# speedinghzl/DSRG

Measured on AMD Instinct MI355X. Metric: images/sec DSRG train step (VGG16 321x321, 21-class), higher is better.
Workload: dtype bf16 backbone (fp32 master weights) + f32/f64 supervision path

## Files before the change

dsrg_amd/_lib.py:

```python
import ctypes
import os

import torch

_HERE = os.path.dirname(os.path.abspath(__file__))
LIB_PATH = os.path.join(_HERE, os.environ.get("DSRG_LIB") or "libdsrg_hip.so")

OK, ERR_INVALID, ERR_HIP, ERR_UNSUPPORTED, ERR_NOMEM = 0, -1, -2, -3, -4


class DsrgError(RuntimeError):
    def __init__(self, code, msg):
        RuntimeError.__init__(self, "libdsrg_hip error %d: %s" % (code, msg))
        self.code = code


class CrfParams(ctypes.Structure):
    _fields_ = [("w_bilateral", ctypes.c_float), ("theta_alpha_x", ctypes.c_float),
                ("theta_alpha_y", ctypes.c_float), ("theta_beta_r", ctypes.c_float),
                ("theta_beta_g", ctypes.c_float), ("theta_beta_b", ctypes.c_float),
                ("w_gaussian", ctypes.c_float), ("theta_gamma_x", ctypes.c_float),
                ("theta_gamma_y", ctypes.c_float), ("n_iters", ctypes.c_int32)]

    @classmethod
# ... 61 lines not shown
    "dsrg_conv_igemm_residual_bf16": (_i, [_vp] * 6 + [_i] * 8 + [_vp]),
    "dsrg_conv_igemm_split_f32": (_i, [_vp, _vp, _vp, _vp] + [_i] * 8 + [_vp]),
    "dsrg_add_relu_bf16": (_i, [_vp, _vp, _vp, _sz, _vp]),
    "dsrg_relu_mask_bf16": (_i, [_vp, _vp, _vp, _vp, _sz, _vp]),
    "dsrg_bias_grad_bf16": (_i, [_vp, _vp, _vp, _i, ctypes.c_long, _i, _vp]),
    "dsrg_heads_forward_bf16": (_i, [_vp, _i, _vp, _vp, _vp, _i, _i, _i, _i, _vp]),
    "dsrg_conv3x3_direct_bf16": (_i, [_vp, _vp, _vp, _vp, _i, _i, _i, _i, _i, _i, _vp]),
    "dsrg_conv3x3_direct_dgrad_workspace": (_sz, [_i]),
    "dsrg_conv3x3_direct_dgrad_bf16": (_i, [_vp] * 6 + [_sz] + [_i] * 5 + [_vp]),
    "dsrg_conv_igemm_supported": (_i, [_i, _i, _i]),
    "dsrg_conv_igemm_bf16": (_i, [_vp, _vp, _vp, _vp, _vp, _i, _i, _i, _i, _i, _i, _i, _i, ctypes.c_float, ctypes.c_ulonglong, _vp, _sz,
                                  _vp]),
    "dsrg_conv_igemm_workspace": (_sz, []),
    "dsrg_conv_igemm_dgrad_workspace": (_sz, [_i] * 5),
    "dsrg_conv_igemm_dgrad_bf16": (_i, [_vp] * 6 + [_i] * 7 + [_f, _vp, _sz, _vp]),
    "dsrg_conv_igemm_workspace_status": (_i, [_vp, _vp, _vp]),
    "dsrg_pack_conv_weight_f32": (_i, [_vp, _vp, _vp, _i, _i, _i, _vp]),
    "dsrg_sgd_pack_f32": (_i, [_i] + [_vp] * 9 + [_f, _vp]),
    "dsrg_conv_igemm_wgrad_workspace": (_sz, [_i, _i, _i, _i, _i, _i, _i]),
    "dsrg_conv_igemm_wgrad_bf16": (_i, [_vp, _vp, _vp, _vp, _i, _vp, _sz, _i, _i, _i, _i, _i, _i, _i, _vp]),
    "dsrg_conv_igemm_backward_bf16": (_i, [_vp, _vp, _vp, _vp, _vp, _vp, _i, _vp, _f, _vp, ctypes.c_size_t, _vp, ctypes.c_size_t, _i, _i, _i, _i, _i, _i, _vp]),
    "dsrg_conv3x3_wgrad_workspace": (_sz, [_i, _i, _i, _i, _i]),
    "dsrg_conv3x3_wgrad_bf16": (_i, [_vp, _vp, _vp, _vp, _sz, _i, _i, _i, _i, _i, _vp]),
    "dsrg_conv3x3_wgrad_f32": (_i, [_vp, _vp, _vp, _vp, _sz, _i, _i, _i, _i, _i, _vp]),
    "dsrg_pack_conv_weight_direct_f32": (_i, [_vp, _vp, _vp, _i, _i, _vp]),
    "dsrg_heads_backward_chunks": (_i, [_i]),
    "dsrg_heads_backward_bf16": (_i, [_vp, _i, _vp, _vp, _vp, _sz, _vp, _vp, _i, _i, _i, _i, _vp]),
    "dsrg_heads_backward_relu_workspace": (_sz, [_i] * 3),
    "dsrg_heads_backward_relu_bf16": (_i, [_vp, _i, _vp, _vp, _vp, _sz, _vp, _vp, _f, _vp, _vp, _sz] + [_i] * 4 + [_vp]),
    "dsrg_maxpool3x3_fwd_bf16": (_i, [_vp, _vp, _vp, _i, _i, _i, _i, _i, _i, _i, _vp]),
    "dsrg_maxpool3x3_relu_fwd_bf16": (_i, [_vp, _vp, _vp, _i, _i, _i, _i, _i, _i, _i, _vp]),
    "dsrg_maxpool3x3_bwd_bf16": (_i, [_vp, _vp, _vp, _i, _i, _i, _i, _i, _i, _i, _vp]),
    "dsrg_maxpool3x3_bwd_relu_bf16": (_i, [_vp, _vp, _vp, _vp, _vp, _vp, _i, _i, _i, _i, _i, _i, _i, _vp]),
    "dsrg_supervision_step": (_i, [_vp, _i, _vp, _vp, _i, _i, _vp, _vp, _d, _d, ctypes.POINTER(CrfParams),
                                   _vp, _vp, _vp, _vp, _vp, _vp]),
}

_LIB = None


def lib():
    global _LIB
    if _LIB is None:
        if not os.path.exists(LIB_PATH):
            raise ImportError(
                "%s is missing — build it with `make -C dsrg_amd/csrc` (hipcc --offload-arch=gfx950) or "
                "`python -c 'import __graft_entry__ as g; g.build()'`.  There is no CPU fallback." % LIB_PATH)
        L = ctypes.CDLL(LIB_PATH)
        for name, (res, args) in SIGNATURES.items():
            fn = getattr(L, name)
            fn.restype = res
            fn.argtypes = args
        _LIB = L
    return _LIB


def check(rc):
    if rc != OK:
        raise DsrgError(rc, lib().dsrg_last_error().decode("utf-8", "replace"))


def require_gpu():
    if lib().dsrg_device_count() < 1:
        raise DsrgError(ERR_HIP, "no HIP device visible — the DSRG supervision kernels need an MI355X "
                                 "(gfx950); there is no CPU fallback")
```

dsrg_amd/backbone.py:

```python
import torch
import torch.nn as nn
import torch.nn.functional as F

import os as _os

from . import ops

_WGRAD_MIN_COUT = 512
_GEMM_DGRAD_MAX_MAP = 2048
_GEMM_WGRAD_MAX_MAP = 2048
_IGEMM_MIN_TILES = 64
_IGEMM = _os.environ.get("DSRG_IGEMM", "1") == "1"


def _bf16_run(x):
    return x.dtype == torch.bfloat16 or (torch.is_autocast_enabled() and torch.get_autocast_dtype("cuda") == torch.bfloat16)


def _im2col_gemm(x, weight, bias, dilation, relu, want_cols=False):
    B, C, H, W = x.shape
    cout, k = weight.shape[0], weight.shape[2]
    xn = x.permute(0, 2, 3, 1)
    if not xn.is_contiguous():
        xn = xn.contiguous()
# ... 132 lines not shown

class _GradLink:
    __slots__ = ("scale", "gb", "ptr", "version")

    def __init__(self):
        self.scale, self.gb, self.ptr, self.version = 1.0, None, 0, -1

    def leave(self, gx, gb):
        self.gb, self.ptr, self.version = gb, gx.data_ptr(), gx._version

    def take(self, g):
        gb, self.gb = self.gb, None
        if gb is None:
            return None
        if g.data_ptr() == self.ptr and g._version == self.version:
            return gb
        if self.scale != 1.0:
            raise RuntimeError("chain_input: the output of a conv + ReLU + Dropout node declared to have one consumer has several")
        return None


_FUSE_CHAIN = _os.environ.get("DSRG_FUSE_CHAIN", "1") != "0"


def _landed(g, slot):
    return g.detach() if (slot is not None and g is slot) else g


class _IgemmConvFn(torch.autograd.Function):

    @staticmethod
    def forward(ctx, k, dils, relu, drop_p, pool, n, links_in, links_out, *t):
        xs, ws, bs = t[:n], t[n:2 * n], t[2 * n:3 * n]
        xs = [x if x.dtype == torch.bfloat16 else x.bfloat16() for x in xs]
        packs_d = [None] * n
        fb = [b.detach().float().contiguous() for b in bs]
        if drop_p > 0.0 and not relu:
            raise ValueError("_IgemmConvFn: Dropout needs the ReLU in front of it")
        fused_drop = drop_p > 0.0
        scale = 256.0 / (256 - min(255, int(drop_p * 256.0 + 0.5))) if fused_drop else 1.0
        seed = ops.dropout_seed() if fused_drop else 0
        if links_in is not None and not all(lk is not None for lk in links_in):
            links_in = None
        if k == 3:
            need_d = any(ctx.needs_input_grad[8:8 + n]) and ops.conv_igemm_supported(ws[0].shape[0], ws[0].shape[1], 3)
            packs = [ops.pack_conv_weight_pair(w, True, need_d) for w in ws]
            packs_d = [p[1] for p in packs]
            outs = ops.conv_igemm(xs, [p[0] for p in packs], fb, dils, 3, relu, drop_p, seed)
        elif fused_drop:
            packs = [ops.pack_conv_weight_pair(w, True, links_in is not None and _FUSE_CHAIN) for w in ws]
            packs_d = [p[1] for p in packs]
            outs = ops.conv_igemm(xs, [p[0] for p in packs], fb, dils, 1, relu, drop_p, seed)
        else:
            outs = [_im2col_gemm(x, w.to(torch.bfloat16), b.to(torch.bfloat16), 1, relu) for x, w, b in zip(xs, ws, bs)]
        code, pooled = None, None
        if pool is not None:
            pooled, code = ops.maxpool3x3_fwd(outs[0], pool[0], pool[1], relu_input=True)
        ctx.save_for_backward(code, *xs, *ws, *(outs if (relu and pool is None) else ()))
        ctx.out_shape = tuple(outs[0].shape)
        ctx.gw_out = [getattr(w, "_dsrg_grad_out", None) for w in ws]
        ctx.packs_d = packs_d
        ctx.dils, ctx.relu, ctx.scale, ctx.pool, ctx.n, ctx.k = dils, relu, scale, pool, n, k
        ctx.links_in = links_in
        ctx.links_out = links_out if (relu and pool is None) else None
        if ctx.links_out is not None:
            for lk in ctx.links_out:
                lk.scale, lk.gb = scale, None
        return tuple(outs) if pool is None else (pooled,)

    @staticmethod
    def backward(ctx, *gs):
        n = ctx.n
        code, saved = ctx.saved_tensors[0], ctx.saved_tensors[1:]
        xs, ws, ys = saved[:n], saved[n:2 * n], saved[2 * n:] or (None,) * n
        cout, cin = ws[0].shape[0], ws[0].shape[1]
        gms, gbs = [], []
        cl = torch.channels_last
        for i, g in enumerate(gs):
            gm, gb = g, ctx.links_out[i].take(g) if ctx.links_out is not None else None
            if gb is None:
                gm, gb = _relu_bias_backward(g, ctx.pool, code, ctx.out_shape, ctx.relu, ys[i], ctx.scale)
            gms.append(gm); gbs.append(gb)
        need_x = [ctx.needs_input_grad[8 + i] for i in range(n)]
        gxs = [None] * n
        absorb = _FUSE_CHAIN and ctx.links_in is not None and all(need_x) and ops.conv_igemm_supported(cout, cin, ctx.k) and \
            cin >= 256 and all(x.is_contiguous(memory_format=cl) for x in xs)
        if n == 1 and ctx.k == 3 and need_x[0] and ops.conv_igemm_supported(cout, cin, 3) and \
                ops.conv_igemm_wgrad_supported(cin, cout, 3) and xs[0].is_contiguous(memory_format=cl):
            pd = ctx.packs_d[0] if ctx.packs_d[0] is not None else ops.pack_conv_weight(ws[0], for_dgrad=True)
            gx, gw, gb_below = ops.conv_igemm_backward(gms[0], pd, xs[0], ctx.dils[0], xs[0] if absorb else None,
                                                       ctx.links_in[0].scale if absorb else 1.0, gw_out=ctx.gw_out[0])
            if absorb:
                ctx.links_in[0].leave(gx, gb_below)
            return (None,) * 8 + (gx, _landed(gw, ctx.gw_out[0])) + tuple(gbs)
        if absorb:
            packs_d = [p if p is not None else ops.pack_conv_weight(w, for_dgrad=True) for p, w in zip(ctx.packs_d, ws)]
            gxs, gb_below = ops.conv_igemm_dgrad(gms, packs_d, list(xs), ctx.dils, ctx.k, ctx.links_in[0].scale)
            for lk, gx_, gb_ in zip(ctx.links_in, gxs, gb_below):
                lk.leave(gx_, gb_)
        if ctx.k == 1:
            for i in range(n):
                if absorb:
                    break
                if need_x[i]:
# ... 125 lines not shown
            if igemm:
                (out,) = _IgemmConvFn.apply(3, [self.dilation[0]], self.fuse_relu, p, node_pool, 1, [lin] if lin is not None else None,
                                            [lout] if lout is not None else None, x, self.weight, self.bias)
            elif direct:
                out = _DirectConvFn.apply(x, self.weight, self.bias, self.fuse_relu, node_pool, lin, lout)
            else:
                out = _ConvFn.apply(x, self.weight, self.bias, self.dilation[0], self.fuse_relu, self.gemm, p, node_pool, lin, lout)
            if lout is not None:
                out._dsrg_grad_link = lout
            return out if pool is None or in_node else _pool3x3(out, pool[0], pool[1])
        out = super().forward(x)
        out = F.relu(out) if self.fuse_relu else out
        out = F.dropout(out, p, True) if p > 0.0 else out
        return out if pool is None else _pool3x3(out, pool[0], pool[1])


class FusedReLU(nn.Identity):
    """placeholder that keeps the Sequential indices (and state_dict keys) of the conv/ReLU pairs: the ReLU itself
    runs inside the GemmConv2d in front of it"""


class FusedPool(nn.Identity):
    """placeholder for the max-pool layer that runs inside the GemmConv2d two slots in front of it (`fuse_pool`)"""


class FusedDropout(nn.Identity):
    """placeholder for the Dropout layer that runs inside the GemmConv2d two slots in front of it (`fuse_dropout`)"""


def _hip_pool_takes(x):
    return x.is_cuda and x.dtype == torch.bfloat16 and x.shape[1] % 8 == 0 and x.is_contiguous(memory_format=torch.channels_last)


class _MaxPool3x3Fn(torch.autograd.Function):
    @staticmethod
    def forward(ctx, x, stride, ceil_mode):
        out, code = ops.maxpool3x3_fwd(x, stride, ceil_mode)
        ctx.save_for_backward(code)
        ctx.in_shape, ctx.stride = x.shape, stride
        return out

    @staticmethod
    def backward(ctx, g):
        (code,) = ctx.saved_tensors
        return ops.maxpool3x3_bwd(g, code, ctx.in_shape, ctx.stride), None, None


class _AvgPool3x3Fn(torch.autograd.Function):
    @staticmethod
    def forward(ctx, x):
        return ops.avgpool3x3_s1(x)

    @staticmethod
    def backward(ctx, g):
        return ops.avgpool3x3_s1(g)


class AvgPool3x3(nn.AvgPool2d):

    def __init__(self):
        super().__init__(3, 1, 1)

    def forward(self, x):
        if _hip_pool_takes(x):
            return _AvgPool3x3Fn.apply(x)
        if x.is_cuda and x.dim() == 4 and not x.is_contiguous():
            x = x.contiguous()
        return super().forward(x)


class MaxPool3x3(nn.MaxPool2d):

    def __init__(self, stride, ceil_mode=False):
        super().__init__(3, stride, 1, ceil_mode=ceil_mode)

    def forward(self, x):
        return _pool3x3(x, self.stride, self.ceil_mode)

# ... 16 lines not shown
        cl = torch.channels_last
        ctx.links = links if (links is not None and all(lk is not None for lk in links) and
                              all(x.is_contiguous(memory_format=cl) for x in xs)) else None
        xs = [x.contiguous(memory_format=cl) for x in xs]
        weight = weight.contiguous()
        ctx.save_for_backward(weight, *xs)
        return ops.heads_forward(xs, weight, bias.contiguous())

    @staticmethod
    def backward(ctx, g):
        weight, *xs = ctx.saved_tensors
        n, O, K = weight.shape
        if _FUSE_CHAIN and ctx.links is not None and all(ctx.needs_input_grad[3:]):
            gxs, gw, gb_below = ops.heads_backward(xs, weight, g, True, ctx.links[0].scale)
            for i, lk in enumerate(ctx.links):
                lk.leave(gxs[i], gb_below[i])
        else:
            gxs, gw = ops.heads_backward(xs, weight, g, need_gx=any(ctx.needs_input_grad[3:]))
        gb1 = g.sum((0, 2, 3))
        return (None, gw, gb1.unsqueeze(0).expand(n, O).contiguous()) + (tuple(gxs) if gxs is not None else (None,) * n)


class _StackKernels(torch.autograd.Function):

    @staticmethod
    def forward(ctx, *ws):
        ctx.layouts = [(tuple(w.shape), tuple(w.stride())) for w in ws]
        return torch.stack([w.reshape(w.shape[0], w.shape[1]) for w in ws])

    @staticmethod
    def backward(ctx, g):
        return tuple(g[i].as_strided(shape, stride) if g[i].is_contiguous() else g[i].reshape(shape)
                     for i, (shape, stride) in enumerate(ctx.layouts))


class VGG16ASPP(nn.Module):

    def __init__(self, num_classes=21, dropout=0.5, gemm_convs=True):
        super().__init__()
        L = []
        p2 = (2, True)
        L += _conv_relu(3, 64) + _conv_relu(64, 64, pool=p2, chain=True)
        L += _conv_relu(64, 128, 1, gemm_convs) + _conv_relu(128, 128, 1, gemm_convs, pool=p2, chain=True)
        L += _conv_relu(128, 256, 1, gemm_convs) + _conv_relu(256, 256, 1, gemm_convs, chain=True) + \
            _conv_relu(256, 256, 1, gemm_convs, pool=p2, chain=True)
        g = gemm_convs
        L += _conv_relu(256, 512, 1, g) + _conv_relu(512, 512, 1, g, chain=True) + _conv_relu(512, 512, 1, g, chain=True) + [MaxPool3x3(1)]
        L += _conv_relu(512, 512, 2, g) + _conv_relu(512, 512, 2, g, chain=True) + _conv_relu(512, 512, 2, g, chain=True) + [MaxPool3x3(1)]
        L += [AvgPool3x3()]
        self.features = nn.Sequential(*L)
        self.branches = nn.ModuleList()
        for d in (6, 12, 18, 24):
            g = gemm_convs
            fc8 = GemmConv2d(1024, num_classes, 1, gemm=g)
            nn.init.normal_(fc8.weight, std=0.01)
            nn.init.zeros_(fc8.bias)
            self.branches.append(nn.Sequential(
                GemmConv2d(512, 1024, 3, padding=d, dilation=d, fuse_relu=True, gemm=g, fuse_dropout=dropout), FusedReLU(),
                FusedDropout(),
                GemmConv2d(1024, 1024, 1, fuse_relu=True, gemm=g, fuse_dropout=dropout), FusedReLU(), FusedDropout(), fc8))

    def forward(self, x):
        f = self.features(x)
        hs = []
        fc6 = [br[0] for br in self.branches]
        if len(fc6) <= 4 and all(_igemm_route(m, f, len(fc6)) and m.stride == (1, 1) and m.padding == m.dilation for m in fc6):
            p = fc6[0].fuse_dropout if self.training else 0.0
            n = len(fc6)
            links = [_GradLink() for _ in range(n)] if torch.is_grad_enabled() else None
            hs = list(_IgemmConvFn.apply(3, [m.dilation[0] for m in fc6], True, p, None, n, None, links, *([f] * n),
                                         *[m.weight for m in fc6], *[m.bias for m in fc6]))
            fc7 = [br[3] for br in self.branches]
            if all(isinstance(m, GemmConv2d) and m.kernel_size == (1, 1) and m.fuse_relu and m.bias is not None and m.gemm
                   and m.in_channels % 256 == 0 and m.out_channels % 256 == 0 for m in fc7):
                p7 = fc7[0].fuse_dropout if self.training else 0.0
                links7 = [_GradLink() for _ in range(n)] if torch.is_grad_enabled() else None
                hs = list(_IgemmConvFn.apply(1, [1] * n, True, p7, None, n, links, links7, *hs, *[m.weight for m in fc7],
                                             *[m.bias for m in fc7]))
                for h, lk in zip(hs, links7 or []):
                    h._dsrg_grad_link = lk
            else:
                for i, br in enumerate(self.branches):
                    for m in list(br)[1:-1]:
                        hs[i] = m(hs[i])
        else:
            for br in self.branches:
                h = f
                for m in list(br)[:-1]:
                    h = m(h)
                hs.append(h)
        heads = [br[-1] for br in self.branches]
        if hs[0].is_cuda and hs[0].dtype == torch.bfloat16 and len(hs) <= 4 and heads[0].out_channels <= 32 \
                and heads[0].in_channels % 256 == 0:
            w = _StackKernels.apply(*[m.weight for m in heads])
            b = torch.stack([m.bias for m in heads])
            links = [getattr(h, "_dsrg_grad_link", None) for h in hs]
            return _HeadsFn.apply(links, w.float(), b.float(), *hs)
        out = None
        with torch.autocast(device_type=hs[0].device.type, enabled=False):
            for m, h in zip(heads, hs):
                s = m(h.float())
                out = s if out is None else out + s
        return out

# ... 49 lines not shown
```

dsrg_amd/ops.py:

```python
import ctypes
import threading

import torch

from . import _lib
from ._lib import CrfParams, check


def _stream():
    return ctypes.c_void_p(torch.cuda.current_stream().cuda_stream)


def _ptr(t):
    return ctypes.c_void_p(t.data_ptr()) if t is not None else None


def _f32c(t, name):
    if not (t.is_cuda and t.dtype == torch.float32 and t.is_contiguous()):
        raise ValueError("%s must be a contiguous float32 CUDA tensor" % name)
    return t


_defer = [False]
_defer_keep = []
# ... 973 lines not shown
        return [gx[k].permute(0, 3, 1, 2) for k in range(n)], gw, gb
    check(L.dsrg_heads_backward_bf16(ptrs, n, _ptr(weight), _ptr(g), _ptr(gx), M * K * 2, _ptr(gw), _ptr(part), B, H * W, K, O,
                                     _stream()))
    return ([gx[k].permute(0, 3, 1, 2) for k in range(n)] if need_gx else None), gw


def maxpool3x3_out_size(n, stride, ceil_mode):
    num = n + 2 - 3
    o = (-(-num // stride) if ceil_mode else num // stride) + 1
    if (o - 1) * stride >= n + 1:
        o -= 1
    return o


def maxpool3x3_fwd(x, stride, ceil_mode, relu_input=False):
    B, C, H, W = x.shape
    OH, OW = maxpool3x3_out_size(H, stride, ceil_mode), maxpool3x3_out_size(W, stride, ceil_mode)
    out = torch.empty((B, C, OH, OW), dtype=x.dtype, device=x.device, memory_format=torch.channels_last)
    code = torch.empty((B, OH, OW, C), dtype=torch.uint8, device=x.device)
    fn = _lib.lib().dsrg_maxpool3x3_relu_fwd_bf16 if relu_input else _lib.lib().dsrg_maxpool3x3_fwd_bf16
    check(fn(_ptr(x), _ptr(out), _ptr(code), B, H, W, OH, OW, C, stride, _stream()))
    return out, code


def maxpool3x3_bwd(gout, code, in_shape, stride):
    B, C, H, W = in_shape
    OH, OW = gout.shape[2], gout.shape[3]
    gout = gout.contiguous(memory_format=torch.channels_last)
    gin = torch.empty((B, C, H, W), dtype=gout.dtype, device=gout.device, memory_format=torch.channels_last)
    check(_lib.lib().dsrg_maxpool3x3_bwd_bf16(_ptr(gout), _ptr(code), _ptr(gin), B, H, W, OH, OW, C, stride, _stream()))
    return gin


def maxpool3x3_bwd_relu(gout, code, relu_out, stride=2, gb_out=None):
    have_y = torch.is_tensor(relu_out)
    B, C, H, W = relu_out.shape if have_y else relu_out
    OH, OW = gout.shape[2], gout.shape[3]
    cl = torch.channels_last
    if stride != 2 or not (gout.is_cuda and gout.dtype == torch.bfloat16 and C % 8 == 0 and 256 % (C // 8) == 0) or (
            have_y and not (relu_out.is_cuda and relu_out.dtype == torch.bfloat16 and relu_out.is_contiguous(memory_format=cl))):
        raise ValueError("maxpool3x3_bwd_relu: stride 2, bf16 channels_last, channels / 8 a divisor of 256")
    gout = gout.contiguous(memory_format=cl)
    gin = torch.empty((B, C, H, W), dtype=torch.bfloat16, device=gout.device, memory_format=cl)
    gb = _dest(gb_out, (C,), torch.float32, gout.device)
    part = _partial_rows(gout.device, C)
    check(_lib.lib().dsrg_maxpool3x3_bwd_relu_bf16(_ptr(gout), _ptr(code), _ptr(relu_out) if have_y else None, _ptr(gin), _ptr(gb), _ptr(part),
                                                   _PARTIAL_BLOCKS, B, H, W, OH, OW, C, _stream()))
    return gin, gb


class DSRGSupervision(torch.autograd.Function):

    @staticmethod
    def forward(ctx, logits, images, labels, cues, th1, th2, scale_factor, maxiter, prepared=False):
        losses, grad, _ = supervision_step(logits.contiguous(), images, labels, cues, th1, th2, scale_factor, maxiter,
                                           prepared=prepared)
        ctx.save_for_backward(grad)
        ctx.mark_non_differentiable(losses)
        return losses.sum(), losses

    @staticmethod
    def backward(ctx, g_total, _g_losses):
        (grad,) = ctx.saved_tensors
        return grad * g_total, None, None, None, None, None, None, None, None


# ... 4 lines not shown
```

include/dsrg_hip.h:

```cpp
#ifndef DSRG_HIP_H
#define DSRG_HIP_H

#include <stddef.h>
#include <stdint.h>

#ifdef __cplusplus
extern "C" {
#endif

#pragma GCC visibility push(default)

#define DSRG_OK 0
#define DSRG_ERR_INVALID (-1)
#define DSRG_ERR_HIP (-2)
#define DSRG_ERR_UNSUPPORTED (-3)
#define DSRG_ERR_NOMEM (-4)

const char *dsrg_last_error(void);
int dsrg_device_count(void);
int dsrg_host_register(void *host, size_t bytes);
int dsrg_host_unregister(void *host);

typedef struct dsrg_crf_s *dsrg_crf_t;

// ... 134 lines not shown
                      float momentum, void *stream);
size_t dsrg_conv_igemm_wgrad_workspace(int ngroups, int B, int H, int W, int cin, int cout, int ksize);
int dsrg_conv_igemm_wgrad_bf16(const void *const *x_dev, const void *const *g_dev, void *const *gw_dev, const int *dilation,
                               int ngroups, void *workspace_dev, size_t workspace_bytes, int B, int H, int W, int cin, int cout,
                               int ksize, int out_bf16, void *stream);
int dsrg_conv_igemm_backward_bf16(const void *g_dev, const void *w_dgrad_dev, const void *x_dev, const void *mask_dev, void *gx_dev,
                                  float *gw_dev, int dilation, float *bias_grad_dev, float mask_scale, void *colsum_workspace_dev,
                                  size_t colsum_workspace_bytes, void *wgrad_workspace_dev, size_t wgrad_workspace_bytes, int B, int H,
                                  int W, int cin, int cout, int ksize, void *stream);
int dsrg_conv_igemm_backward_residual_bf16(const void *g_dev, const void *w_dgrad_dev, const void *x_dev, const void *mask_dev,
                                           const void *res_dev, void *gx_dev, float *gw_dev, const float *gw_scale_dev, int dilation,
                                           void *wgrad_workspace_dev, size_t wgrad_workspace_bytes, int B, int H, int W, int cin, int cout,
                                           int ksize, void *stream);
int dsrg_heads_forward_bf16(const void *const *x_dev, int n_branches, const float *w_dev, const float *bias_dev,
                            float *out_dev, int B, int HW, int K, int O, void *stream);
int dsrg_heads_backward_chunks(int M);
int dsrg_heads_backward_bf16(const void *const *x_dev, int n_branches, const float *w_dev, const float *g_dev,
                             void *gx_dev, size_t gx_branch_stride_bytes, float *gw_dev, float *partial_dev, int B,
                             int HW, int K, int O, void *stream);
size_t dsrg_heads_backward_relu_workspace(int n_branches, int M, int K);
int dsrg_heads_backward_relu_bf16(const void *const *x_dev, int n_branches, const float *w_dev, const float *g_dev,
                                  void *gx_dev, size_t gx_branch_stride_bytes, float *gw_dev, float *partial_dev,
                                  float relu_scale, float *bias_grad_dev, void *workspace_dev, size_t workspace_bytes, int B,
                                  int HW, int K, int O, void *stream);
int dsrg_maxpool3x3_fwd_bf16(const void *in_dev, void *out_dev, void *code_dev, int B, int H, int W, int OH, int OW, int C,
                             int stride, void *stream);
int dsrg_maxpool3x3_relu_fwd_bf16(const void *in_dev, void *out_dev, void *code_dev, int B, int H, int W, int OH, int OW, int C,
                                  int stride, void *stream);
int dsrg_maxpool3x3_bwd_bf16(const void *gout_dev, const void *code_dev, void *gin_dev, int B, int H, int W, int OH, int OW,
                             int C, int stride, void *stream);
int dsrg_maxpool3x3_bwd_relu_bf16(const void *gout_dev, const void *code_dev, const void *relu_out_dev, void *gin_dev,
                                  float *bias_grad_dev, float *partials_dev, int partial_blocks, int B, int H, int W, int OH,
                                  int OW, int C, void *stream);

int dsrg_supervision_step(dsrg_ctx_t ctx, int B, const float *logits_dev, const float *images_dev,
                          int img_h, int img_w, const float *labels_dev, const float *cues_dev,
                          double th1, double th2, const dsrg_crf_params *params,
                          float *losses_dev, float *grad_logits_dev,
                          float *probs_dev, float *seeds_dev, float *logq_dev, void *stream);

#pragma GCC visibility pop

#ifdef __cplusplus
}
#endif
#endif
```

Measured before the change: 1958.

## Fuse final stride-1 maxpool and avgpool with LDS-tiled kernels and branch-gradient sum

Adds LDS-tiled HIP kernels for the stride-1 3x3 maxpool, plus a fused maxpool-then-avgpool forward and backward for the end of the feature stack. In backward, the four ASPP branch input gradients are passed straight to the fused pool backward through a link object instead of being summed by autograd, so the separate sum and pool passes over HBM go away. The cost is extra bookkeeping that can fall back when a gradient was modified in place, plus LDS-size limits that trigger the old path.

```diff
diff --git a/dsrg_amd/_lib.py b/dsrg_amd/_lib.py
--- a/dsrg_amd/_lib.py
+++ b/dsrg_amd/_lib.py
@@ -117,6 +117,11 @@
     "dsrg_maxpool3x3_relu_fwd_bf16": (_i, [_vp, _vp, _vp, _i, _i, _i, _i, _i, _i, _i, _vp]),
     "dsrg_maxpool3x3_bwd_bf16": (_i, [_vp, _vp, _vp, _i, _i, _i, _i, _i, _i, _i, _vp]),
     "dsrg_maxpool3x3_bwd_relu_bf16": (_i, [_vp, _vp, _vp, _vp, _vp, _vp, _i, _i, _i, _i, _i, _i, _i, _vp]),
+    "dsrg_pool_chain_rows": (_i, []),
+    "dsrg_maxpool3x3_s1_tiled_fwd_bf16": (_i, [_vp, _vp, _vp, _i, _i, _i, _i, _vp]),
+    "dsrg_maxavg3x3_s1_fwd_bf16": (_i, [_vp, _vp, _vp, _i, _i, _i, _i, _vp]),
+    "dsrg_maxpool3x3_s1_tiled_bwd_bf16": (_i, [_vp, _vp, _vp, _i, _i, _i, _i, _vp]),
+    "dsrg_maxavg3x3_s1_bwd_bf16": (_i, [_vp, _vp, _vp, _vp, _i, _vp, _vp, _i, _i, _i, _i, _vp]),
     "dsrg_supervision_step": (_i, [_vp, _i, _vp, _vp, _i, _i, _vp, _vp, _d, _d, ctypes.POINTER(CrfParams),
                                    _vp, _vp, _vp, _vp, _vp, _vp]),
 }
diff --git a/dsrg_amd/backbone.py b/dsrg_amd/backbone.py
--- a/dsrg_amd/backbone.py
+++ b/dsrg_amd/backbone.py
@@ -188,6 +188,8 @@
     @staticmethod
     def forward(ctx, k, dils, relu, drop_p, pool, n, links_in, links_out, *t):
         xs, ws, bs = t[:n], t[n:2 * n], t[2 * n:3 * n]
+        ctx.extra = len(t) - 3 * n
+        ctx.sum_link = t[3 * n] if ctx.extra else None
         xs = [x if x.dtype == torch.bfloat16 else x.bfloat16() for x in xs]
         packs_d = [None] * n
         fb = [b.detach().float().contiguous() for b in bs]
@@ -226,6 +228,16 @@
 
     @staticmethod
     def backward(ctx, *gs):
+        res = _IgemmConvFn._backward(ctx, *gs)
+        n, lk = ctx.n, ctx.sum_link
+        gxs = res[8:8 + n]
+        if lk is not None and _POOL_CHAIN and n > 1 and all(g is not None and _hip_pool_takes(g) for g in gxs):
+            lk.leave(gxs)
+            res = res[:9] + (None,) * (n - 1) + res[8 + n:]
+        return res + (None,) * ctx.extra
+
+    @staticmethod
+    def _backward(ctx, *gs):
         n = ctx.n
         code, saved = ctx.saved_tensors[0], ctx.saved_tensors[1:]
         xs, ws, ys = saved[:n], saved[n:2 * n], saved[2 * n:] or (None,) * n
@@ -417,10 +429,16 @@
     return x.is_cuda and x.dtype == torch.bfloat16 and x.shape[1] % 8 == 0 and x.is_contiguous(memory_format=torch.channels_last)
 
 
+_POOL_CHAIN = _os.environ.get("DSRG_POOL_CHAIN", "1") != "0"
+
+
 class _MaxPool3x3Fn(torch.autograd.Function):
     @staticmethod
     def forward(ctx, x, stride, ceil_mode):
-        out, code = ops.maxpool3x3_fwd(x, stride, ceil_mode)
+        if stride == 1 and _POOL_CHAIN:
+            out, code = ops.maxpool3x3_s1_tiled_fwd(x, ctx.needs_input_grad[0])
+        else:
+            out, code = ops.maxpool3x3_fwd(x, stride, ceil_mode)
         ctx.save_for_backward(code)
         ctx.in_shape, ctx.stride = x.shape, stride
         return out
@@ -428,7 +446,48 @@
     @staticmethod
     def backward(ctx, g):
         (code,) = ctx.saved_tensors
+        if ctx.stride == 1 and _POOL_CHAIN and _hip_pool_takes(g):
+            return ops.maxpool3x3_s1_tiled_bwd(g, code), None, None
         return ops.maxpool3x3_bwd(g, code, ctx.in_shape, ctx.stride), None, None
+
+
+class _SumLink:
+    __slots__ = ("gs", "ptr", "version")
+
+    def __init__(self):
+        self.gs, self.ptr, self.version = None, 0, -1
+
+    def leave(self, gs):
+        self.gs, self.ptr, self.version = list(gs), gs[0].data_ptr(), gs[0]._version
+
+    def take(self, g):
+        gs, self.gs = self.gs, None
+        if gs is None:
+            return [g], True
+        if g.data_ptr() == self.ptr and g._version == self.version and g.shape == gs[0].shape and g.dtype == gs[0].dtype:
+            return gs, True
+        return [g] + gs[1:], False
+
+
+class _PoolChainFn(torch.autograd.Function):
+
+    @staticmethod
+    def forward(ctx, x, link):
+        out, code = ops.maxavg3x3_s1_fwd(x, ctx.needs_input_grad[0])
+        ctx.save_for_backward(code)
+        ctx.in_shape, ctx.link = x.shape, link
+        return out
+
+    @staticmethod
+    def backward(ctx, g):
+        (code,) = ctx.saved_tensors
+        gs, intact = ctx.link.take(g) if ctx.link is not None else ([g], True)
+        if intact and _POOL_CHAIN and all(_hip_pool_takes(t) for t in gs):
+            return ops.maxavg3x3_s1_bwd(gs, code), None
+        s = gs[0]
+        for t in gs[1:]:
+            s = s + t
+        return ops.maxpool3x3_bwd(ops.avgpool3x3_s1(s), code, ctx.in_shape, 1), None
 
 
 class _AvgPool3x3Fn(torch.autograd.Function):
@@ -511,6 +570,24 @@
     def backward(ctx, g):
         return tuple(g[i].as_strided(shape, stride) if g[i].is_contiguous() else g[i].reshape(shape)
                      for i, (shape, stride) in enumerate(ctx.layouts))
+
+
+class _Features(nn.Sequential):
+
+    def forward(self, x):
+        mods = list(self)
+        if not (_POOL_CHAIN and len(mods) >= 2 and isinstance(mods[-2], MaxPool3x3) and mods[-2].stride == 1
+                and isinstance(mods[-1], AvgPool3x3)):
+            return super().forward(x)
+        for m in mods[:-2]:
+            x = m(x)
+        if not _hip_pool_takes(x):
+            return mods[-1](mods[-2](x))
+        link = _SumLink() if (torch.is_grad_enabled() and x.requires_grad) else None
+        out = _PoolChainFn.apply(x, link)
+        if link is not None:
+            out._dsrg_sum_link = link
+        return out
 
 
 class VGG16ASPP(nn.Module):
@@ -527,7 +604,7 @@
         L += _conv_relu(256, 512, 1, g) + _conv_relu(512, 512, 1, g, chain=True) + _conv_relu(512, 512, 1, g, chain=True) + [MaxPool3x3(1)]
         L += _conv_relu(512, 512, 2, g) + _conv_relu(512, 512, 2, g, chain=True) + _conv_relu(512, 512, 2, g, chain=True) + [MaxPool3x3(1)]
         L += [AvgPool3x3()]
-        self.features = nn.Sequential(*L)
+        self.features = _Features(*L)
         self.branches = nn.ModuleList()
         for d in (6, 12, 18, 24):
             g = gemm_convs
@@ -547,8 +624,10 @@
             p = fc6[0].fuse_dropout if self.training else 0.0
             n = len(fc6)
             links = [_GradLink() for _ in range(n)] if torch.is_grad_enabled() else None
+            sum_link = getattr(f, "_dsrg_sum_link", None) if (_POOL_CHAIN and n > 1) else None
             hs = list(_IgemmConvFn.apply(3, [m.dilation[0] for m in fc6], True, p, None, n, None, links, *([f] * n),
-                                         *[m.weight for m in fc6], *[m.bias for m in fc6]))
+                                         *[m.weight for m in fc6], *[m.bias for m in fc6],
+                                         *([sum_link] if sum_link is not None else [])))
             fc7 = [br[3] for br in self.branches]
             if all(isinstance(m, GemmConv2d) and m.kernel_size == (1, 1) and m.fuse_relu and m.bias is not None and m.gemm
                    and m.in_channels % 256 == 0 and m.out_channels % 256 == 0 for m in fc7):
diff --git a/dsrg_amd/csrc/pool_chain.hip b/dsrg_amd/csrc/pool_chain.hip
--- /dev/null
+++ b/dsrg_amd/csrc/pool_chain.hip
@@ -0,0 +1,391 @@
+#include "common.h"
+#include <algorithm>
+
+#ifndef DSRG_POOL_ROWS
+#define DSRG_POOL_ROWS 8
+#endif
+
+namespace dsrg {
+namespace {
+
+constexpr int kPoolRows = DSRG_POOL_ROWS;
+constexpr int kSegRows = 4;
+constexpr int kMaxThreads = 1024;
+constexpr size_t kLdsLimit = 160 * 1024;
+
+__device__ __forceinline__ float lo16(uint32_t w) { return __uint_as_float(w << 16); }
+__device__ __forceinline__ float hi16(uint32_t w) { return __uint_as_float(w & 0xffff0000u); }
+__device__ __forceinline__ uint32_t to_bf16(float f) {
+    uint32_t u = __float_as_uint(f);
+    if ((u & 0x7fffffffu) > 0x7f800000u) return (u >> 16) | 0x40u;
+    return (u + 0x7fffu + ((u >> 16) & 1u)) >> 16;
+}
+__device__ __forceinline__ uint32_t pack2(float lo, float hi) { return to_bf16(lo) | (to_bf16(hi) << 16); }
+__device__ __forceinline__ uint32_t to_bf16_torch(float f) {
+    uint32_t u = __float_as_uint(f);
+    if (f != f) return 0x7fc0u;
+    return (u + 0x7fffu + ((u >> 16) & 1u)) >> 16;
+}
+__device__ __forceinline__ uint32_t add_pair(uint32_t a, uint32_t b) {
+    return to_bf16_torch(lo16(a) + lo16(b)) | (to_bf16_torch(hi16(a) + hi16(b)) << 16);
+}
+__device__ __forceinline__ uint4 add_vec(uint4 a, uint4 b) {
+    return make_uint4(add_pair(a.x, b.x), add_pair(a.y, b.y), add_pair(a.z, b.z), add_pair(a.w, b.w));
+}
+
+struct Tile {
+    int b, y0, y1;
+    int cg0, cga;
+    int H, W, C8;
+};
+__device__ __forceinline__ Tile make_tile(int H, int W, int C8, int CG) {
+    Tile t;
+    t.b = blockIdx.z;
+    t.y0 = blockIdx.x * kPoolRows;
+    t.y1 = min(H, t.y0 + kPoolRows);
+    t.cg0 = blockIdx.y * CG;
+    t.cga = min(CG, C8 - t.cg0);
+    t.H = H; t.W = W; t.C8 = C8;
+    return t;
+}
+
+template <typename T>
+__device__ __forceinline__ void stage_rows(T *lds, const T *__restrict__ g, const Tile &t, int ra, int rb, int base) {
+    ra = max(ra, 0); rb = min(rb, t.H);
+    const int lanes = blockDim.x / t.cga, c = threadIdx.x % t.cga, p0 = threadIdx.x / t.cga;
+    if (p0 >= lanes) return;
+    const int npix = (rb - ra) * t.W;
+    const T *src = g + ((size_t)t.b * t.H + ra) * t.W * t.C8 + t.cg0 + c;
+    T *dst = lds + (size_t)(ra - base) * t.W * t.cga + c;
+    int p = p0;
+    for (; p + 3 * lanes < npix; p += 4 * lanes) {
+        const T v0 = src[(size_t)p * t.C8], v1 = src[(size_t)(p + lanes) * t.C8];
+        const T v2 = src[(size_t)(p + 2 * lanes) * t.C8], v3 = src[(size_t)(p + 3 * lanes) * t.C8];
+        dst[p * t.cga] = v0; dst[(p + lanes) * t.cga] = v1; dst[(p + 2 * lanes) * t.cga] = v2; dst[(p + 3 * lanes) * t.cga] = v3;
+    }
+    for (; p < npix; p += lanes) dst[p * t.cga] = src[(size_t)p * t.C8];
+}
+
+__device__ __forceinline__ void stage_sum_rows(uint4 *lds, const uint4 *__restrict__ g0, const uint4 *__restrict__ g1,
+                                               const uint4 *__restrict__ g2, const uint4 *__restrict__ g3, int n, const Tile &t,
+                                               int ra, int rb, int base) {
+    ra = max(ra, 0); rb = min(rb, t.H);
+    const int lanes = blockDim.x / t.cga, c = threadIdx.x % t.cga, p0 = threadIdx.x / t.cga;
+    if (p0 >= lanes) return;
+    const int npix = (rb - ra) * t.W;
+    const size_t off = ((size_t)t.b * t.H + ra) * t.W * t.C8 + t.cg0 + c;
+    uint4 *dst = lds + (size_t)(ra - base) * t.W * t.cga + c;
+    for (int p = p0; p < npix; p += lanes) {
+        const size_t i = off + (size_t)p * t.C8;
+        uint4 s = g0[i];
+        if (n > 1) {
+            const uint4 a = g1[i];
+            if (n > 2) {
+                const uint4 b2 = g2[i];
+                if (n > 3) {
+                    const uint4 b3 = g3[i];
+                    s = add_vec(add_vec(add_vec(s, a), b2), b3);
+                } else {
+                    s = add_vec(add_vec(s, a), b2);
+                }
+            } else {
+                s = add_vec(s, a);
+            }
+        }
+        dst[p * t.cga] = s;
+    }
+}
+
+struct Task { int c, x, ys, ye; };
+__device__ __forceinline__ int task_count(const Tile &t, int ra, int rb) { return ((rb - ra + kSegRows - 1) / kSegRows) * t.W * t.cga; }
+__device__ __forceinline__ Task make_task(const Tile &t, int i, int ra, int rb) {
+    Task k;
+    k.c = i % t.cga;
+    const int q = i / t.cga;
+    k.x = q % t.W;
+    k.ys = ra + (q / t.W) * kSegRows;
+    k.ye = min(rb, k.ys + kSegRows);
+    return k;
+}
+
+struct RowMax { float v[8]; uint32_t c[8]; };
+__device__ __forceinline__ void row_max(const uint4 *row, int x, int W, int cga, int c, RowMax &r) {
+#pragma unroll
+    for (int k = 0; k < 8; ++k) { r.v[k] = -__builtin_inff(); r.c[k] = 0xffu; }
+#pragma unroll
+    for (int dx = 0; dx < 3; ++dx) {
+        const int xx = x - 1 + dx;
+        if (xx < 0 || xx >= W) continue;
+        const uint4 v = row[xx * cga + c];
+        const uint32_t w[4] = {v.x, v.y, v.z, v.w};
+#pragma unroll
+        for (int k = 0; k < 4; ++k) {
+            const float lo = lo16(w[k]), hi = hi16(w[k]);
+            if (lo > r.v[2 * k] || lo != lo || r.c[2 * k] == 0xffu) { r.v[2 * k] = lo; r.c[2 * k] = dx; }
+            if (hi > r.v[2 * k + 1] || hi != hi || r.c[2 * k + 1] == 0xffu) { r.v[2 * k + 1] = hi; r.c[2 * k + 1] = dx; }
+        }
+    }
+}
+__device__ __forceinline__ void fold_row(const RowMax &r, int dy, float *best, uint32_t *bc) {
+#pragma unroll
+    for (int k = 0; k < 8; ++k)
+        if (r.v[k] > best[k] || r.v[k] != r.v[k] || bc[k] == 0xffu) { best[k] = r.v[k]; bc[k] = 3 * dy + r.c[k]; }
+}
+
+template <bool TO_LDS>
+__device__ __forceinline__ void maxpool_rows(const uint4 *in_l, int in_base, const Tile &t, int ra, int rb, uint4 *out_g, uint4 *out_l,
+                                             int out_base, uint2 *code, int ca, int cb) {
+    const int W = t.W, cga = t.cga, H = t.H, ntask = task_count(t, ra, rb);
+    for (int i = threadIdx.x; i < ntask; i += blockDim.x) {
+        const Task k = make_task(t, i, ra, rb);
+        RowMax r0, r1, r2;
+        if (k.ys > 0) row_max(in_l + (size_t)(k.ys - 1 - in_base) * W * cga, k.x, W, cga, k.c, r0);
+        row_max(in_l + (size_t)(k.ys - in_base) * W * cga, k.x, W, cga, k.c, r1);
+        for (int y = k.ys; y < k.ye; ++y) {
+            if (y + 1 < H) row_max(in_l + (size_t)(y + 1 - in_base) * W * cga, k.x, W, cga, k.c, r2);
+            float best[8];
+            uint32_t bc[8];
+#pragma unroll
+            for (int j = 0; j < 8; ++j) { best[j] = -__builtin_inff(); bc[j] = 0xffu; }
+            if (y > 0) fold_row(r0, 0, best, bc);
+            fold_row(r1, 1, best, bc);
+            if (y + 1 < H) fold_row(r2, 2, best, bc);
+            const uint4 o = make_uint4(pack2(best[0], best[1]), pack2(best[2], best[3]), pack2(best[4], best[5]), pack2(best[6], best[7]));
+            const size_t gi = (((size_t)t.b * H + y) * W + k.x) * t.C8 + t.cg0 + k.c;
+            if (TO_LDS) out_l[((size_t)(y - out_base) * W + k.x) * cga + k.c] = o;
+            else out_g[gi] = o;
+            if (code && y >= ca && y < cb)
+                code[gi] = make_uint2(bc[0] | (bc[1] << 8) | (bc[2] << 16) | (bc[3] << 24), bc[4] | (bc[5] << 8) | (bc[6] << 16) | (bc[7] << 24));
+            r0 = r1; r1 = r2;
+        }
+    }
+}
+
+__device__ __forceinline__ void load_taps(const uint4 *row, int x, int W, int cga, int c, uint4 *w) {
+    if (x > 0) w[0] = row[(x - 1) * cga + c];
+    w[1] = row[x * cga + c];
+    if (x + 1 < W) w[2] = row[(x + 1) * cga + c];
+}
+__device__ __forceinline__ void load_taps(const uint2 *row, int x, int W, int cga, int c, uint2 *w) {
+    if (x > 0) w[0] = row[(x - 1) * cga + c];
+    w[1] = row[x * cga + c];
+    if (x + 1 < W) w[2] = row[(x + 1) * cga + c];
+}
+__device__ __forceinline__ void add_taps(const uint4 *w, bool left, bool right, float *acc) {
+#pragma unroll
+    for (int dx = 0; dx < 3; ++dx) {
+        if ((dx == 0 && !left) || (dx == 2 && !right)) continue;
+        const uint32_t u[4] = {w[dx].x, w[dx].y, w[dx].z, w[dx].w};
+#pragma unroll
+        for (int k = 0; k < 4; ++k) { acc[2 * k] += lo16(u[k]); acc[2 * k + 1] += hi16(u[k]); }
+    }
+}
+
+template <bool TO_LDS>
+__device__ __forceinline__ void avgpool_rows(const uint4 *in_l, int in_base, const Tile &t, int ra, int rb, uint4 *out_g, uint4 *out_l,
+                                             int out_base) {
+    const int W = t.W, cga = t.cga, H = t.H, ntask = task_count(t, ra, rb);
+    for (int i = threadIdx.x; i < ntask; i += blockDim.x) {
+        const Task k = make_task(t, i, ra, rb);
+        const bool left = k.x > 0, right = k.x + 1 < W;
+        uint4 w0[3], w1[3], w2[3];
+        w0[0] = w0[1] = w0[2] = w1[0] = w1[1] = w1[2] = w2[0] = w2[1] = w2[2] = make_uint4(0u, 0u, 0u, 0u);
+        if (k.ys > 0) load_taps(in_l + (size_t)(k.ys - 1 - in_base) * W * cga, k.x, W, cga, k.c, w0);
+        load_taps(in_l + (size_t)(k.ys - in_base) * W * cga, k.x, W, cga, k.c, w1);
+        for (int y = k.ys; y < k.ye; ++y) {
+            if (y + 1 < H) load_taps(in_l + (size_t)(y + 1 - in_base) * W * cga, k.x, W, cga, k.c, w2);
+            float acc[8] = {0.f, 0.f, 0.f, 0.f, 0.f, 0.f, 0.f, 0.f};
+            if (y > 0) add_taps(w0, left, right, acc);
+            add_taps(w1, left, right, acc);
+            if (y + 1 < H) add_taps(w2, left, right, acc);
+#pragma unroll
+            for (int j = 0; j < 8; ++j) acc[j] = acc[j] / 9.0f;
+            const uint4 o = make_uint4(pack2(acc[0], acc[1]), pack2(acc[2], acc[3]), pack2(acc[4], acc[5]), pack2(acc[6], acc[7]));
+            if (TO_LDS) out_l[((size_t)(y - out_base) * W + k.x) * cga + k.c] = o;
+            else out_g[(((size_t)t.b * H + y) * W + k.x) * t.C8 + t.cg0 + k.c] = o;
+#pragma unroll
+            for (int j = 0; j < 3; ++j) { w0[j] = w1[j]; w1[j] = w2[j]; }
+        }
+    }
+}
+
+__device__ __forceinline__ void gather_taps(const uint4 *g, const uint2 *cd, int dy, bool left, bool right, float *acc) {
+#pragma unroll
+    for (int dx = 0; dx < 3; ++dx) {
+        if ((dx == 0 && !right) || (dx == 2 && !left)) continue;
+        const uint4 gv = g[2 - dx];
+        const uint2 cv = cd[2 - dx];
+        const uint32_t want = 3 * dy + dx;
+        const uint32_t gw[4] = {gv.x, gv.y, gv.z, gv.w};
+#pragma unroll
+        for (int k = 0; k < 4; ++k) {
+            const uint32_t cw = k < 2 ? cv.x : cv.y;
+            const uint32_t c0 = (cw >> (16 * (k & 1))) & 0xffu, c1 = (cw >> (16 * (k & 1) + 8)) & 0xffu;
+            if (c0 == want) acc[2 * k] += lo16(gw[k]);
+            if (c1 == want) acc[2 * k + 1] += hi16(gw[k]);
+        }
+    }
+}
+
+__device__ __forceinline__ void maxpool_bwd_rows(const uint4 *g_l, const uint2 *c_l, int base, const Tile &t, int ra, int rb, uint4 *gin) {
+    const int W = t.W, cga = t.cga, H = t.H, ntask = task_count(t, ra, rb);
+    for (int i = threadIdx.x; i < ntask; i += blockDim.x) {
+        const Task k = make_task(t, i, ra, rb);
+        const bool left = k.x > 0, right = k.x + 1 < W;
+        uint4 g0[3], g1[3], g2[3];
+        uint2 c0[3], c1[3], c2[3];
+        g0[0] = g0[1] = g0[2] = g1[0] = g1[1] = g1[2] = g2[0] = g2[1] = g2[2] = make_uint4(0u, 0u, 0u, 0u);
+        c0[0] = c0[1] = c0[2] = c1[0] = c1[1] = c1[2] = c2[0] = c2[1] = c2[2] = make_uint2(0u, 0u);
+        if (k.ys > 0) {
+            load_taps(g_l + (size_t)(k.ys - 1 - base) * W * cga, k.x, W, cga, k.c, g0);
+            load_taps(c_l + (size_t)(k.ys - 1 - base) * W * cga, k.x, W, cga, k.c, c0);
+        }
+        load_taps(g_l + (size_t)(k.ys - base) * W * cga, k.x, W, cga, k.c, g1);
+        load_taps(c_l + (size_t)(k.ys - base) * W * cga, k.x, W, cga, k.c, c1);
+        for (int y = k.ys; y < k.ye; ++y) {
+            if (y + 1 < H) {
+                load_taps(g_l + (size_t)(y + 1 - base) * W * cga, k.x, W, cga, k.c, g2);
+                load_taps(c_l + (size_t)(y + 1 - base) * W * cga, k.x, W, cga, k.c, c2);
+            }
+            float acc[8] = {0.f, 0.f, 0.f, 0.f, 0.f, 0.f, 0.f, 0.f};
+            if (y + 1 < H) gather_taps(g2, c2, 0, left, right, acc);
+            gather_taps(g1, c1, 1, left, right, acc);
+            if (y > 0) gather_taps(g0, c0, 2, left, right, acc);
+            gin[(((size_t)t.b * H + y) * W + k.x) * t.C8 + t.cg0 + k.c] =
+                make_uint4(pack2(acc[0], acc[1]), pack2(acc[2], acc[3]), pack2(acc[4], acc[5]), pack2(acc[6], acc[7]));
+#pragma unroll
+            for (int j = 0; j < 3; ++j) { g0[j] = g1[j]; g1[j] = g2[j]; c0[j] = c1[j]; c1[j] = c2[j]; }
+        }
+    }
+}
+
+extern __shared__ uint4 pool_lds[];
+
+__global__ __launch_bounds__(kMaxThreads) void maxpool3x3_s1_tiled_fwd_kernel(const uint4 *__restrict__ in, uint4 *__restrict__ out,
+                                                                                uint2 *__restrict__ code, int H, int W, int C8, int CG) {
+    const Tile t = make_tile(H, W, C8, CG);
+    const int base = t.y0 - 1;
+    stage_rows(pool_lds, in, t, t.y0 - 1, t.y1 + 1, base);
+    __syncthreads();
+    maxpool_rows<false>(pool_lds, base, t, t.y0, t.y1, out, nullptr, 0, code, t.y0, t.y1);
+}
+
+__global__ __launch_bounds__(kMaxThreads) void maxavg3x3_s1_fwd_kernel(const uint4 *__restrict__ in, uint4 *__restrict__ out,
+                                                                         uint2 *__restrict__ code, int H, int W, int C8, int CG) {
+    const Tile t = make_tile(H, W, C8, CG);
+    const int base = t.y0 - 2, pbase = t.y0 - 1;
+    uint4 *pooled = pool_lds + (size_t)(kPoolRows + 4) * W * t.cga;
+    stage_rows(pool_lds, in, t, t.y0 - 2, t.y1 + 2, base);
+    __syncthreads();
+    maxpool_rows<true>(pool_lds, base, t, max(t.y0 - 1, 0), min(t.y1 + 1, H), nullptr, pooled, pbase, code, t.y0, t.y1);
+    __syncthreads();
+    avgpool_rows<false>(pooled, pbase, t, t.y0, t.y1, out, nullptr, 0);
+}
+
+__global__ __launch_bounds__(kMaxThreads) void maxpool3x3_s1_tiled_bwd_kernel(const uint4 *__restrict__ gout, const uint2 *__restrict__ code,
+                                                                                uint4 *__restrict__ gin, int H, int W, int C8, int CG) {
+    const Tile t = make_tile(H, W, C8, CG);
+    const int base = t.y0 - 1;
+    uint2 *codes = reinterpret_cast<uint2 *>(pool_lds + (size_t)(kPoolRows + 2) * W * t.cga);
+    stage_rows(pool_lds, gout, t, t.y0 - 1, t.y1 + 1, base);
+    stage_rows(codes, code, t, t.y0 - 1, t.y1 + 1, base);
+    __syncthreads();
+    maxpool_bwd_rows(pool_lds, codes, base, t, t.y0, t.y1, gin);
+}
+
+__global__ __launch_bounds__(kMaxThreads) void maxavg3x3_s1_bwd_kernel(const uint4 *__restrict__ g0, const uint4 *__restrict__ g1,
+                                                                         const uint4 *__restrict__ g2, const uint4 *__restrict__ g3, int n,
+                                                                         const uint2 *__restrict__ code, uint4 *__restrict__ gin, int H,
+                                                                         int W, int C8, int CG) {
+    const Tile t = make_tile(H, W, C8, CG);
+    const int base = t.y0 - 2, abase = t.y0 - 1;
+    uint4 *avg = pool_lds + (size_t)(kPoolRows + 4) * W * t.cga;
+    uint2 *codes = reinterpret_cast<uint2 *>(avg + (size_t)(kPoolRows + 2) * W * t.cga);
+    stage_rows(codes, code, t, t.y0 - 1, t.y1 + 1, abase);
+    stage_sum_rows(pool_lds, g0, g1, g2, g3, n, t, t.y0 - 2, t.y1 + 2, base);
+    __syncthreads();
+    avgpool_rows<true>(pool_lds, base, t, max(t.y0 - 1, 0), min(t.y1 + 1, H), nullptr, avg, abase);
+    __syncthreads();
+    maxpool_bwd_rows(avg, codes, abase, t, t.y0, t.y1, gin);
+}
+
+struct Geometry { int CG; size_t lds; dim3 grid; int threads; };
+int plan(const char *what, int B, int H, int W, int C, int rows16, int rows8, int walk_rows, Geometry &g) {
+    if (C % 8 != 0) return set_error(DSRG_ERR_UNSUPPORTED, "%s: channels must be a multiple of 8", what);
+    if (B <= 0 || H <= 0 || W <= 0 || B > 65535) return set_error(DSRG_ERR_INVALID, "%s: bad shape", what);
+    const int C8 = C / 8;
+    int CG = 8;
+    while (CG > 1 && CG / 2 >= C8) CG /= 2;
+    for (;; CG /= 2) {
+        g.lds = (size_t)W * CG * ((size_t)rows16 * 16 + (size_t)rows8 * 8);
+        if (g.lds <= kLdsLimit) break;
+        if (CG == 1) return set_error(DSRG_ERR_UNSUPPORTED, "%s: a strip of %d-pixel rows does not fit in LDS", what, W);
+    }
+    g.CG = CG;
+    const int strips = (H + kPoolRows - 1) / kPoolRows, blocks = (C8 + CG - 1) / CG;
+    if (blocks > 65535) return set_error(DSRG_ERR_UNSUPPORTED, "%s: too many channel blocks", what);
+    g.grid = dim3(strips, blocks, B);
+    const long tasks = (long)((walk_rows + kSegRows - 1) / kSegRows) * W * CG;
+    g.threads = (int)std::min<long>(kMaxThreads, (tasks + 63) / 64 * 64);
+    return DSRG_OK;
+}
+
+}
+}
+
+using namespace dsrg;
+
+extern "C" int dsrg_pool_chain_rows(void) { return kPoolRows; }
+
+extern "C" int dsrg_maxpool3x3_s1_tiled_fwd_bf16(const void *in, void *out, void *code, int B, int H, int W, int C, void *stream) {
+    if (!in || !out) return set_error(DSRG_ERR_INVALID, "NULL argument");
+    Geometry g;
+    if (int rc = plan("maxpool3x3_s1_tiled_fwd", B, H, W, C, kPoolRows + 2, 0, kPoolRows, g)) return rc;
+    static LdsGrant grant;
+    if (int rc = ensure_dynamic_lds(reinterpret_cast<const void *>(&maxpool3x3_s1_tiled_fwd_kernel), g.lds, grant)) return rc;
+    hipLaunchKernelGGL(maxpool3x3_s1_tiled_fwd_kernel, g.grid, dim3(g.threads), g.lds, static_cast<hipStream_t>(stream), (const uint4 *)in,
+                       (uint4 *)out, (uint2 *)code, H, W, C / 8, g.CG);
+    DSRG_LAUNCH_CHECK();
+    return DSRG_OK;
+}
+
+extern "C" int dsrg_maxavg3x3_s1_fwd_bf16(const void *in, void *out, void *code, int B, int H, int W, int C, void *stream) {
+    if (!in || !out) return set_error(DSRG_ERR_INVALID, "NULL argument");
+    Geometry g;
+    if (int rc = plan("maxavg3x3_s1_fwd", B, H, W, C, 2 * kPoolRows + 6, 0, kPoolRows + 2, g)) return rc;
+    static LdsGrant grant;
+    if (int rc = ensure_dynamic_lds(reinterpret_cast<const void *>(&maxavg3x3_s1_fwd_kernel), g.lds, grant)) return rc;
+    hipLaunchKernelGGL(maxavg3x3_s1_fwd_kernel, g.grid, dim3(g.threads), g.lds, static_cast<hipStream_t>(stream), (const uint4 *)in,
+                       (uint4 *)out, (uint2 *)code, H, W, C / 8, g.CG);
+    DSRG_LAUNCH_CHECK();
+    return DSRG_OK;
+}
+
+extern "C" int dsrg_maxpool3x3_s1_tiled_bwd_bf16(const void *gout, const void *code, void *gin, int B, int H, int W, int C, void *stream) {
+    if (!gout || !code || !gin) return set_error(DSRG_ERR_INVALID, "NULL argument");
+    Geometry g;
+    if (int rc = plan("maxpool3x3_s1_tiled_bwd", B, H, W, C, kPoolRows + 2, kPoolRows + 2, kPoolRows, g)) return rc;
+    static LdsGrant grant;
+    if (int rc = ensure_dynamic_lds(reinterpret_cast<const void *>(&maxpool3x3_s1_tiled_bwd_kernel), g.lds, grant)) return rc;
+    hipLaunchKernelGGL(maxpool3x3_s1_tiled_bwd_kernel, g.grid, dim3(g.threads), g.lds, static_cast<hipStream_t>(stream), (const uint4 *)gout,
+                       (const uint2 *)code, (uint4 *)gin, H, W, C / 8, g.CG);
+    DSRG_LAUNCH_CHECK();
+    return DSRG_OK;
+}
+
+extern "C" int dsrg_maxavg3x3_s1_bwd_bf16(const void *g0, const void *g1, const void *g2, const void *g3, int n, const void *code,
+                                          void *gin, int B, int H, int W, int C, void *stream) {
+    if (n < 1 || n > 4) return set_error(DSRG_ERR_INVALID, "maxavg3x3_s1_bwd: 1 to 4 gradients");
+    const void *gs[4] = {g0, g1, g2, g3};
+    for (int i = 0; i < n; ++i)
+        if (!gs[i]) return set_error(DSRG_ERR_INVALID, "NULL argument");
+    if (!code || !gin) return set_error(DSRG_ERR_INVALID, "NULL argument");
+    Geometry g;
+    if (int rc = plan("maxavg3x3_s1_bwd", B, H, W, C, 2 * kPoolRows + 6, kPoolRows + 2, kPoolRows + 2, g)) return rc;
+    static LdsGrant grant;
+    if (int rc = ensure_dynamic_lds(reinterpret_cast<const void *>(&maxavg3x3_s1_bwd_kernel), g.lds, grant)) return rc;
+    hipLaunchKernelGGL(maxavg3x3_s1_bwd_kernel, g.grid, dim3(g.threads), g.lds, static_cast<hipStream_t>(stream), (const uint4 *)g0,
+                       (const uint4 *)g1, (const uint4 *)g2, (const uint4 *)g3, n, (const uint2 *)code, (uint4 *)gin, H, W, C / 8, g.CG);
+    DSRG_LAUNCH_CHECK();
+    return DSRG_OK;
+}
diff --git a/dsrg_amd/ops.py b/dsrg_amd/ops.py
--- a/dsrg_amd/ops.py
+++ b/dsrg_amd/ops.py
@@ -1029,6 +1029,73 @@
     return gin
 
 
+def __getattr__(name):
+    if name == "POOL_CHAIN_ROWS":
+        return int(_lib.lib().dsrg_pool_chain_rows())
+    raise AttributeError("module %r has no attribute %r" % (__name__, name))
+
+
+def _fits(rc):
+    if rc == _lib.ERR_UNSUPPORTED:
+        return False
+    check(rc)
+    return True
+
+
+def _cl_bf16(t, what):
+    if not (t.is_cuda and t.dtype == torch.bfloat16 and t.dim() == 4 and t.shape[1] % 8 == 0):
+        raise ValueError("%s: a (B,C,H,W) bf16 CUDA tensor with 8 | C" % what)
+    return t.contiguous(memory_format=torch.channels_last)
+
+
+def maxpool3x3_s1_tiled_fwd(x, want_code=True):
+    x = _cl_bf16(x, "maxpool3x3_s1_tiled_fwd")
+    B, C, H, W = x.shape
+    out = torch.empty_like(x)
+    code = torch.empty((B, H, W, C), dtype=torch.uint8, device=x.device) if want_code else None
+    if _fits(_lib.lib().dsrg_maxpool3x3_s1_tiled_fwd_bf16(_ptr(x), _ptr(out), _ptr(code), B, H, W, C, _stream())):
+        return out, code
+    out, code = maxpool3x3_fwd(x, 1, False)
+    return out, (code if want_code else None)
+
+
+def maxavg3x3_s1_fwd(x, want_code=True):
+    x = _cl_bf16(x, "maxavg3x3_s1_fwd")
+    B, C, H, W = x.shape
+    out = torch.empty_like(x)
+    code = torch.empty((B, H, W, C), dtype=torch.uint8, device=x.device) if want_code else None
+    if _fits(_lib.lib().dsrg_maxavg3x3_s1_fwd_bf16(_ptr(x), _ptr(out), _ptr(code), B, H, W, C, _stream())):
+        return out, code
+    pooled, code = maxpool3x3_fwd(x, 1, False)
+    return avgpool3x3_s1(pooled), (code if want_code else None)
+
+
+def maxpool3x3_s1_tiled_bwd(gout, code):
+    gout = _cl_bf16(gout, "maxpool3x3_s1_tiled_bwd")
+    B, C, H, W = gout.shape
+    gin = torch.empty_like(gout)
+    if _fits(_lib.lib().dsrg_maxpool3x3_s1_tiled_bwd_bf16(_ptr(gout), _ptr(code), _ptr(gin), B, H, W, C, _stream())):
+        return gin
+    return maxpool3x3_bwd(gout, code, gout.shape, 1)
+
+
+def maxavg3x3_s1_bwd(gouts, code):
+    if not 1 <= len(gouts) <= 4:
+        raise ValueError("maxavg3x3_s1_bwd: 1 to 4 gradients")
+    gouts = [_cl_bf16(g, "maxavg3x3_s1_bwd") for g in gouts]
+    if any(g.shape != gouts[0].shape for g in gouts):
+        raise ValueError("maxavg3x3_s1_bwd: gradients of one shape")
+    B, C, H, W = gouts[0].shape
+    gin = torch.empty_like(gouts[0])
+    ptrs = [_ptr(g) for g in gouts] + [None] * (4 - len(gouts))
+    if _fits(_lib.lib().dsrg_maxavg3x3_s1_bwd_bf16(*ptrs, len(gouts), _ptr(code), _ptr(gin), B, H, W, C, _stream())):
+        return gin
+    s = gouts[0]
+    for g in gouts[1:]:
+        s = s + g
+    return maxpool3x3_bwd(avgpool3x3_s1(s), code, gouts[0].shape, 1)
+
+
 def maxpool3x3_bwd_relu(gout, code, relu_out, stride=2, gb_out=None):
     have_y = torch.is_tensor(relu_out)
     B, C, H, W = relu_out.shape if have_y else relu_out
diff --git a/include/dsrg_hip.h b/include/dsrg_hip.h
--- a/include/dsrg_hip.h
+++ b/include/dsrg_hip.h
@@ -190,6 +190,14 @@
 int dsrg_maxpool3x3_bwd_relu_bf16(const void *gout_dev, const void *code_dev, const void *relu_out_dev, void *gin_dev,
                                   float *bias_grad_dev, float *partials_dev, int partial_blocks, int B, int H, int W, int OH,
                                   int OW, int C, void *stream);
+int dsrg_pool_chain_rows(void);
+int dsrg_maxpool3x3_s1_tiled_fwd_bf16(const void *in_dev, void *out_dev, void *code_dev, int B, int H, int W, int C,
+                                      void *stream);
+int dsrg_maxavg3x3_s1_fwd_bf16(const void *in_dev, void *out_dev, void *code_dev, int B, int H, int W, int C, void *stream);
+int dsrg_maxpool3x3_s1_tiled_bwd_bf16(const void *gout_dev, const void *code_dev, void *gin_dev, int B, int H, int W, int C,
+                                      void *stream);
+int dsrg_maxavg3x3_s1_bwd_bf16(const void *g0_dev, const void *g1_dev, const void *g2_dev, const void *g3_dev, int n,
+                               const void *code_dev, void *gin_dev, int B, int H, int W, int C, void *stream);
 
 int dsrg_supervision_step(dsrg_ctx_t ctx, int B, const float *logits_dev, const float *images_dev,
                           int img_h, int img_w, const float *labels_dev, const float *cues_dev,
```

After: 1966, median of 6. No clear change (+0.4%).
